# unixpickle/learn-nerf

Measured on AMD Instinct MI355X. Metric: ray-samples/s (NeRF train step: fwd + bwd + Adam, 4096 rays x 192 samples per GPU), higher is better.
Workload: dtype bf16; 1 GPU; vanilla NeRF coarse64+fine128 train step (BASELINE.json configs[1]); rays_per_gpu=4096, coarse_samples=64, fine_samples=128, global_batch_rays=4096, parallelism=dp1, precision=bf16 MFMA, fp32 accumulate/master weights

## Files before the change

### learn-nerf_amd/csrc/fused_chain.h

```cpp
#pragma once
#include <utility>

#include "common.h"
#include "fast_math.h"
#include "nerf_wgrad.h"

namespace lnrf {
using namespace nl;

typedef __bf16 bf16x8 __attribute__((ext_vector_type(8)));
typedef float f32x16 __attribute__((ext_vector_type(16)));
typedef float f32x4 __attribute__((ext_vector_type(4)));
typedef short s16x4 __attribute__((ext_vector_type(4)));


template <class F, int... I>
__device__ __forceinline__ void static_for_impl(F&& f, std::integer_sequence<int, I...>) {
  (f(std::integral_constant<int, I>{}), ...);
}
template <int N, class F>
__device__ __forceinline__ void static_for(F&& f) {
  static_for_impl(f, std::make_integer_sequence<int, N>{});
}

// ... 173 lines not shown
    w[p] = __builtin_bit_cast(unsigned, b);
  }
  return __builtin_bit_cast(bf16x8, w);
}

__device__ __forceinline__ unsigned relu_bits(const bf16x8& f0, const bf16x8& f1) {
  const uint4 a = frag_to_bits(f0), b = frag_to_bits(f1);
  const unsigned w[8] = {a.x, a.y, a.z, a.w, b.x, b.y, b.z, b.w};
  unsigned bits = 0u;
#pragma unroll
  for (int i = 0; i < 8; ++i) {
    bits |= ((w[i] & 0xFFFFu) != 0u ? 1u : 0u) << (2 * i);
    bits |= ((w[i] >> 16) != 0u ? 1u : 0u) << (2 * i + 1);
  }
  return bits;
}
template <int S>
__device__ __forceinline__ bf16x8 masked_frag(const f32x16& acc, unsigned bits, int shift) {
  bf16x8 f;
#pragma unroll
  for (int j = 0; j < 8; ++j) f[j] = (__bf16)(((bits >> (shift + 8 * S + j)) & 1u) ? acc[8 * S + j] : 0.0f);
  return f;
}

__device__ __forceinline__ void store_tile_row(float* row, int h, const f32x16& acc) {
  float* zr = row + 4 * h;
#pragma unroll
  for (int g = 0; g < 4; ++g)
    *reinterpret_cast<float4*>(zr + 8 * g) = make_float4(acc[4 * g], acc[4 * g + 1], acc[4 * g + 2], acc[4 * g + 3]);
}
__device__ __forceinline__ void stream_store(gchar* p, uint4 v) {
  u32x4 t = {v.x, v.y, v.z, v.w};
  __builtin_nontemporal_store(t, reinterpret_cast<__attribute__((address_space(1))) u32x4*>(p));
}

__device__ __forceinline__ int64_t dump_off(int slot, int64_t tile, int64_t n_tiles, int n_slots) {
  if (n_slots > 0) return (tile * n_slots + slot) * kFragBytes;
  return ((int64_t)slot * n_tiles + tile) * kFragBytes;
}
struct DumpAddr {
  char* base;
  int64_t n_tiles;
  int64_t tile;
  int c, hh;
  int n_slots;
  __device__ __forceinline__ gchar* at(int slot) const {
// ... 78 lines not shown


__device__ __forceinline__ bf16x8 tr_frag(const char* frag_even, int lane, int parity, int q) {
  const int g = lane >> 4;
  const int i = lane & 15;
  const int frag = g & 1;
  const int hk = g >> 1;
  const int qp = i >> 2, p = i & 3;
  const int slot_par = parity ^ frag;
  const int c0 = 16 * q + 8 * hk;
  const int ca = c0 + qp, cb = c0 + 4 + qp;
  const char* base = frag_even + frag * kFragBytes;
  const int offa = 256 * (ca >> 3) + 128 * (((ca >> 2) & 1) ^ slot_par) + 64 * (p & 1) + 16 * (ca & 3) + 8 * (p >> 1);
  const int offb = 256 * (cb >> 3) + 128 * (((cb >> 2) & 1) ^ slot_par) + 64 * (p & 1) + 16 * (cb & 3) + 8 * (p >> 1);
  const s16x4 lo = __builtin_amdgcn_ds_read_tr16_b64_v4i16((__attribute__((address_space(3))) s16x4*)(base + offa));
  const s16x4 hi = __builtin_amdgcn_ds_read_tr16_b64_v4i16((__attribute__((address_space(3))) s16x4*)(base + offb));
  typedef short s16x8 __attribute__((ext_vector_type(8)));
  s16x8 v;
  v[0] = lo[0]; v[1] = lo[1]; v[2] = lo[2]; v[3] = lo[3];
  v[4] = hi[0]; v[5] = hi[1]; v[6] = hi[2]; v[7] = hi[3];
  return __builtin_bit_cast(bf16x8, v);
}

template <int NXF, int NYF, int SPI, bool PLAIN = false>
struct WgStage {
  static constexpr int kWgSpi = SPI;
  static constexpr int NF = NXF + NYF;
  static constexpr int PER_WAVE = (NF + kWaves - 1) / kWaves;
  static constexpr int STEP_BYTES = NF * kFragBytes;
  static constexpr int ITER_BYTES = kWgSpi * STEP_BYTES;
  const char* x_base;
  const char* y_base;
  int x_slot0, y_slot0, x_slots, y_slots;
  int64_t t0, n_tiles;
  int64_t iter_stride, t_end;
  int wave, lane;
  uint4 rr[kWgSpi][PER_WAVE];

  __device__ __forceinline__ void load(int64_t iter) {
    const int64_t tb = t0 + iter * iter_stride;
    const int64_t tbc = tb < t_end ? tb : t0;
    const int64_t xo = dump_off(x_slot0, tbc, n_tiles, x_slots), yo = dump_off(y_slot0, tbc, n_tiles, y_slots);
    const __amdgpu_buffer_rsrc_t rx = __builtin_amdgcn_make_buffer_rsrc(const_cast<char*>(x_base) + xo, 0, 0x7FFFFFFF, 0x00020000);
    const __amdgpu_buffer_rsrc_t ry = __builtin_amdgcn_make_buffer_rsrc(const_cast<char*>(y_base) + yo, 0, 0x7FFFFFFF, 0x00020000);
#pragma unroll
    for (int u = 0; u < kWgSpi; ++u) {
      const int64_t tl = tb + u;
      const bool ok = tl < t_end;
      const int64_t ta = ok ? tl : tbc;
      const unsigned keep = ok ? 0xFFFFFFFFu : 0u;
#pragma unroll
      for (int q = 0; q < PER_WAVE; ++q) {
        int f = wave + kWaves * q;
        if constexpr (NF % kWaves != 0) f = f < NF ? f : NF - 1;
        const bool isx = f < NXF;
        const int bo = (int)(isx ? dump_off(x_slot0 + f, ta, n_tiles, x_slots) - xo
                                 : dump_off(y_slot0 + f - NXF, ta, n_tiles, y_slots) - yo);
        const u32x4 v = __builtin_amdgcn_raw_buffer_load_b128(isx ? rx : ry, bo + lane * 16, 0, PLAIN ? 0 : 2);
        rr[u][q] = make_uint4(v[0] & keep, v[1] & keep, v[2] & keep, v[3] & keep);
      }
    }
  }
  template <int B>
  __device__ __forceinline__ void write() {
#pragma unroll
    for (int u = 0; u < kWgSpi; ++u) {
#pragma unroll
      for (int q = 0; q < PER_WAVE; ++q) {
        int f = wave + kWaves * q;
        if constexpr (NF % kWaves != 0) f = f < NF ? f : NF - 1;
        *reinterpret_cast<uint4*>(&smem[B * ITER_BYTES + u * STEP_BYTES + f * kFragBytes + lane * 16]) = rr[u][q];
      }
    }
  }
};

template <int NXF, int NYF, int WI, int WO, int SPI, bool PLAIN, class PB>
__device__ __forceinline__ void wgrad_body(const PB& pb, const char* __restrict__ save,
                                           const char* __restrict__ gdump, int64_t n_tiles,
                                           WgLayout lay, float* __restrict__ slabs) {
  constexpr int NI = NXF / 2, NO = NYF / 2;
  constexpr int TI = (NI + WI - 1) / WI, TO = (NO + WO - 1) / WO;
  constexpr bool FULL_I = TI * WI == NI, FULL_O = TO * WO == NO;
  using Stage = WgStage<NXF, NYF, SPI, PLAIN>;
  constexpr int kWgSpi = SPI;
  static_assert(WI * WO == kWaves, "wave grid");
  static_assert(NXF % 2 == 0 && NYF % 2 == 0, "fragment pairs");

  const int split = blockIdx.x - pb.first_block;

  const int tid = threadIdx.x;
  const int lane = tid & 63;
  const int wave = __builtin_amdgcn_readfirstlane(tid >> 6);
  const int wi = wave / WO, wo = wave % WO;

  const int64_t per = (n_tiles + pb.n_blocks - 1) / pb.n_blocks;
  int64_t t0 = (int64_t)split * per;
  const int64_t t1 = t0 + per < n_tiles ? t0 + per : n_tiles;
  const int64_t steps = t1 > t0 ? t1 - t0 : 0;
  int64_t iters = (steps + kWgSpi - 1) / kWgSpi;
  int64_t iter_stride = kWgSpi, t_end = t1;
  if (lay.interleave) {
    t0 = (int64_t)split * kWgSpi;
    iter_stride = (int64_t)pb.n_blocks * kWgSpi;
    t_end = n_tiles;
    iters = t0 < n_tiles ? (n_tiles - t0 + iter_stride - 1) / iter_stride : 0;
  }

  Stage stg;
  stg.x_base = save;
  stg.y_base = gdump;
  stg.x_slot0 = pb.x_slot0;
  stg.y_slot0 = pb.y_slot0;
  stg.x_slots = lay.x_slots;
  stg.y_slots = lay.y_slots;
  stg.t0 = t0;
  stg.n_tiles = n_tiles;
  stg.iter_stride = iter_stride;
  stg.t_end = t_end;
  stg.wave = wave;
  stg.lane = lane;

  f32x16 acc[TI][TO];
#pragma unroll
  for (int a = 0; a < TI; ++a)
#pragma unroll
    for (int b = 0; b < TO; ++b) acc[a][b] = zero_acc();
  float bsum[TO];
#pragma unroll
  for (int b = 0; b < TO; ++b) bsum[b] = 0.0f;
  const int ypar = pb.y_slot0 & 1, xpar = pb.x_slot0 & 1;

  auto compute = [&](auto buf_) {
    constexpr int bufi = decltype(buf_)::value;
#pragma unroll
    for (int u = 0; u < kWgSpi; ++u) {
      const char* buf = smem + bufi * Stage::ITER_BYTES + u * Stage::STEP_BYTES;
#pragma unroll
      for (int q = 0; q < 2; ++q) {
        bf16x8 bf[TO];
#pragma unroll
        for (int b = 0; b < TO; ++b) {
          const int ot = wo + WO * b;
          if (FULL_O || ot < NO) {
// ... 130 lines not shown
```

### learn-nerf_amd/csrc/nerf_bwd_ls.hip

```cpp
#include "nerf_chain.h"

namespace lnrf {

constexpr int kLsWaves = 4;
constexpr int kLsThreads = kLsWaves * 64;
constexpr int kLsStages = 8;
constexpr int kLsLag = 2;
constexpr int kLsDist = kLsLag + 1;
constexpr int kLsBufs = kLsDist + 1;
constexpr int kLsTileBytes = 32 * kFragBytes;
constexpr int kLsPollOff = kLsBufs * kLsTileBytes;
constexpr int kLsLds = kLsPollOff + 5 * 256;
constexpr unsigned kLsMaxSpins = 1u << 18;
constexpr int kLsSlabWaveFloats = 16 * kSlabTileFloats + 2 * 64;
constexpr int64_t kLsSlabBlockBytes = (int64_t)kLsWaves * kLsSlabWaveFloats * (int64_t)sizeof(float);
constexpr int kLsCounterStride = 32;

struct LsJob {
  const char* packed;
  const char* save;
  char* gdump;
  unsigned* counters;
  float* slabs;
  unsigned* status;
// ... 380 lines not shown
  if (bid < n_small) {
    const int prob = bid / (kWaves * kSlabMaxTiles), w = bid / kSlabMaxTiles % kWaves, j = bid % kSlabMaxTiles;
    const WgradProblem pb = a.w[k].p[prob];
    switch (pb.shape) {
#define X(name)                                                                                                    \
  case name:                                                                                                       \
    wgrad_reduce_tile<WgShape<name>::NXF, WgShape<name>::NYF, WgShape<name>::WI, WgShape<name>::WO, NerfWgradEpi>( \
        pb, w, j, a.small_slabs[k], a.grads[k], lds);                                                              \
    break;
      LNRF_WGRAD_LS_SHAPES(X, default: X)
#undef X
    }
  } else if (bid - n_small < kLsStages * 64) {
    ls_fold_block<kSlabReduceWaves>(bid - n_small, a.ls_slabs[k], a.pipelines[k], a.grads[k], lds);
  }
}

struct BwdHeadSeq {
  static constexpr int count = bwd_cons_base(2);
  static constexpr int at(int c) { return bwd_seq(c); }
};
constexpr int kBwdHeadStages = bwd_base(2) / kStageFrags;

__global__ __launch_bounds__(kThreads) void nerf_bwd_head_kernel(
    const char* __restrict__ packed, const char* __restrict__ save, const float* __restrict__ density,
    const float* __restrict__ rgb, const float* __restrict__ g_density, const float* __restrict__ g_rgb,
    int64_t M, int64_t n_tiles, char* __restrict__ gdump, unsigned* __restrict__ zero_words, int n_zero_words) {
  const int tid = threadIdx.x;
  const int lane = tid & 63;
  const int wave = __builtin_amdgcn_readfirstlane(tid >> 6);
  const int64_t tile = (int64_t)blockIdx.x * kWaves + wave;
  for (int i = blockIdx.x * kThreads + tid; i < n_zero_words; i += gridDim.x * kThreads) zero_words[i] = 0u;
  Ring<kBwdHeadStages, BwdHeadSeq> ring;
  ring.stream = packed + kPackBwdOff;
  ring.wave = wave;
  ring.lane = lane;
  const DumpAddr gd{gdump, n_tiles, tile, lane & 31, lane >> 5, kGradTileSlots};
  bwd_chain_tile<true>(ring, gd, save, n_tiles, density, rgb, g_density, g_rgb, M, tile, lane);
}

}

using namespace lnrf;

#ifdef LNRF_TIMELINE
extern "C" int lnrf_debug_set_ls_timeline(void* buf) {
  hipError_t e = hipMemcpyToSymbol(HIP_SYMBOL(lnrf::g_ls_timeline_buf), &buf, sizeof(buf));
  return e == hipSuccess ? LNRF_OK : hip_fail(e, "hipMemcpyToSymbol(g_ls_timeline_buf)");
}
#endif

constexpr int kLsMaxPipelines = 64;
static int ls_pipelines_for_device(int need, int* out) {
  int cus = 0;
  if (int rc = cu_count(&cus)) return rc;
  *out = cus / kLsStages < kLsMaxPipelines ? cus / kLsStages : kLsMaxPipelines;
  if (*out < need) {
    set_error("layer-stationary backward: the device has too few CUs for a pipeline of 8 per model");
    return LNRF_ERR_UNSUPPORTED;
  }
  return LNRF_OK;
// ... 41 lines not shown
  a.n_jobs = 1;
  a.total_pipelines = total;
  a.job[0] = a.job[1] = ls_job(packed, save, scratch, m, total);
  hipError_t e = hipMemsetAsync(a.job[0].counters, 0, kLsCounterBytes, st);
  if (e != hipSuccess) return hip_fail(e, "hipMemsetAsync(counters)");
  hipLaunchKernelGGL(nerf_bwd_ls_kernel, dim3((unsigned)(total * kLsStages)), dim3(kLsThreads), kLsLds, st, a);
  LNRF_LAUNCH_CHECK();
  hipLaunchKernelGGL(nerf_ls_reduce_kernel, dim3(kLsStages * 64), dim3(256), 0, st, (const float*)a.job[0].slabs, total, grads);
  LNRF_LAUNCH_CHECK();
  return LNRF_OK;
}

namespace {
struct LsModel {
  const void* packed;
  const void* save;
  const float *density, *rgb, *g_density, *g_rgb;
  int64_t m;
  void* scratch;
  float* grads;
};
}

static int ls_backward(const LsModel* mdl, int n_models, int phases, hipStream_t st) {
  constexpr int kHeadLds = kRingBytes + round_up(kBiasFloats * 4, 1024);
  int total = 0;
  int rc = ls_pipelines_for_device(n_models, &total);
  if (!rc) rc = set_max_dynamic_lds(nerf_bwd_head_kernel, kHeadLds);
  if (!rc) rc = set_max_dynamic_lds(nerf_bwd_ls_kernel, kLsLds);
  if (rc) return rc;
  int pipes[2] = {total, 0};
  if (n_models == 2) {
    const double share = (double)mdl[0].m / (double)(mdl[0].m + mdl[1].m);
    pipes[0] = (int)(total * share + 0.5);
    if (pipes[0] < 1) pipes[0] = 1;
    if (pipes[0] > total - 1) pipes[0] = total - 1;
    pipes[1] = total - pipes[0];
  }
  LsArgs a;
  a.n_jobs = n_models;
  a.total_pipelines = total;
  for (int k = 0; k < n_models; ++k) {
    const LsModel& md = mdl[k];
    const LsJob& j = a.job[k] = ls_job(md.packed, md.save, md.scratch, md.m, pipes[k]);
    if (phases & 1) {
      hipLaunchKernelGGL(nerf_bwd_head_kernel, dim3((unsigned)(j.n_tiles / kWaves)), dim3(kThreads), kHeadLds, st, j.packed,
                         j.save, md.density, md.rgb, md.g_density, md.g_rgb, md.m, j.n_tiles, j.gdump, j.counters,
                         (phases & 2) ? (int)(kLsCounterBytes / sizeof(unsigned)) : 0);
      LNRF_LAUNCH_CHECK();
    }
    if ((phases & 3) == 2) {
      hipError_t e = hipMemsetAsync(j.counters, 0, kLsCounterBytes, st);
      if (e != hipSuccess) return hip_fail(e, "hipMemsetAsync(counters)");
    }
  }
  if (n_models == 1) a.job[1] = a.job[0];
  if (phases & 2) {
    hipLaunchKernelGGL(nerf_bwd_ls_kernel, dim3((unsigned)(total * kLsStages)), dim3(kLsThreads), kLsLds, st, a);
    LNRF_LAUNCH_CHECK();
  }
  if (!(phases & 4)) return LNRF_OK;
  LsFoldArgs fold;
  for (int k = 0; k < n_models; ++k) {
    const LsModel& md = mdl[k];
    const LsJob& j = a.job[k];
    const WgradList w = wgrad_list_ls_finish(j.n_tiles);
    float* small_slabs = ls_small_slabs(md.scratch, md.m);
    rc = launch_nerf_wgrad(w, md.save, md.scratch, j.n_tiles, md.grads, st, WgLayout{kSaveTileSlots, kGradTileSlots, 1},
                           small_slabs, false, false);
    if (rc) return rc;
    fold.w[k] = w.args;
    fold.small_slabs[k] = small_slabs;
    fold.ls_slabs[k] = j.slabs;
    fold.grads[k] = md.grads;
    fold.pipelines[k] = pipes[k];
  }
  if (n_models == 1) {
    fold.w[1] = fold.w[0]; fold.small_slabs[1] = fold.small_slabs[0]; fold.ls_slabs[1] = fold.ls_slabs[0];
    fold.grads[1] = fold.grads[0]; fold.pipelines[1] = fold.pipelines[0];
  }
  const int gx = fold.w[0].n_problems * kWaves * kSlabMaxTiles + kLsStages * 64;
  hipLaunchKernelGGL(nerf_ls_fold_kernel, dim3((unsigned)gx, (unsigned)n_models), dim3(64 * kSlabReduceWaves), 0, st, fold);
  LNRF_LAUNCH_CHECK();
  return LNRF_OK;
}

extern "C" int lnrf_nerf_mlp_bwd_ls(const lnrf_nerf_shape* shape, const void* packed, const void* save,
                                    const float* density, const float* rgb, const float* g_density,
                                    const float* g_rgb, int64_t m, void* scratch, float* grads, int32_t phases,
                                    lnrf_stream_t stream) {
  LNRF_REQUIRE_NERF_SHAPE(shape);
  LNRF_CHECK_ARG(packed && save && density && rgb && g_density && g_rgb && scratch && grads, "null pointer");
  LNRF_CHECK_ARG(m >= 0, "bad m");
  if (m == 0) return LNRF_OK;
  LNRF_CHECK_ARG(phases >= 1 && phases <= 7, "phases: bit 0 head, bit 1 pipeline, bit 2 small problems + fold");
  const LsModel md{packed, save, density, rgb, g_density, g_rgb, m, scratch, grads};
  return ls_backward(&md, 1, phases, as_stream(stream));
}

extern "C" int lnrf_nerf_mlp_bwd_ls2(const lnrf_nerf_shape* shape, const void* packed_a, const void* save_a,
                                     const float* density_a, const float* rgb_a, const float* g_density_a,
                                     const float* g_rgb_a, int64_t m_a, void* scratch_a, float* grads_a,
                                     const void* packed_b, const void* save_b, const float* density_b,
                                     const float* rgb_b, const float* g_density_b, const float* g_rgb_b, int64_t m_b,
                                     void* scratch_b, float* grads_b, int32_t phases, lnrf_stream_t stream) {
  LNRF_REQUIRE_NERF_SHAPE(shape);
  LNRF_CHECK_ARG(packed_a && save_a && density_a && rgb_a && g_density_a && g_rgb_a && scratch_a && grads_a, "null pointer");
  LNRF_CHECK_ARG(packed_b && save_b && density_b && rgb_b && g_density_b && g_rgb_b && scratch_b && grads_b, "null pointer");
  LNRF_CHECK_ARG(m_a > 0 && m_b > 0, "both models need evaluations (use lnrf_nerf_mlp_bwd_ls for one)");
  const LsModel md[2] = {{packed_a, save_a, density_a, rgb_a, g_density_a, g_rgb_a, m_a, scratch_a, grads_a},
                         {packed_b, save_b, density_b, rgb_b, g_density_b, g_rgb_b, m_b, scratch_b, grads_b}};
  LNRF_CHECK_ARG(phases >= 1 && phases <= 7, "phases: bit 0 head, bit 1 pipeline, bit 2 small problems + fold");
  return ls_backward(md, 2, phases, as_stream(stream));
}
```

### learn-nerf_amd/csrc/nerf_chain.h

```cpp
#pragma once
#include "fused_chain.h"

namespace lnrf {

template <class Put>
__device__ __forceinline__ void x_encode(const float (&px)[3], int h, Put put) {
  static_for<4>([&](auto ks_) {
    constexpr int ks = decltype(ks_)::value;
#pragma unroll
    for (int pp = 0; pp < 4; ++pp) {
      const int p = 4 * ks + pp;
      float s = 0.0f, co = 0.0f;
      if (p < kXPairs) {
        const int pg = kXPairs * h + p;
        const int cd = pg / kXFreqs, f = pg - kXFreqs * cd;
        const float v = cd == 0 ? px[0] : (cd == 1 ? px[1] : px[2]);
        sincos_pe(v * (float)(1 << f), &s, &co);
      }
      put(ks_, 2 * pp, s);
      put(ks_, 2 * pp + 1, co);
    }
  });
}

// ... 12 lines not shown
        else return xe[ks - 16];
      },
      epi);
}
template <int S, class RING, class Epi>
__device__ __forceinline__ void trunk_layer_split(RING& ring, int h, const bf16x8 (&xe_hi)[4], const bf16x8 (&xe_lo)[4],
                                                  const bf16x8 (&inh)[16], const bf16x8 (&inl)[16], Epi epi) {
  chain_layer_split<fwd_cons_base(S), fwd_nk(S), fwd_no(S)>(
      ring, [&](auto o_) { return bias_acc(fwd_bias_base(S) + 32 * decltype(o_)::value, h); },
      [&](auto k_) -> bf16x8 {
        constexpr int ks = decltype(k_)::value;
        if constexpr (S == 0) return xe_hi[ks];
        else if constexpr (ks < 16) return inh[ks];
        else return xe_hi[ks - 16];
      },
      [&](auto k_) -> bf16x8 {
        constexpr int ks = decltype(k_)::value;
        if constexpr (S == 0) return xe_lo[ks];
        else if constexpr (ks < 16) return inl[ks];
        else return xe_lo[ks - 16];
      },
      epi);
}
template <int O>
__device__ __forceinline__ void masked_out_tile(const f32x16& acc, const uint4& mk, bf16x8 (&out)[16], const DumpAddr& gd,
                                                int slot0) {
  const unsigned mb = mask_word(mk, O);
  out[2 * O] = masked_frag<0>(acc, mb, 16 * (O & 1));
  out[2 * O + 1] = masked_frag<1>(acc, mb, 16 * (O & 1));
  gd.store(slot0 + 2 * O, frag_to_bits(out[2 * O]));
  gd.store(slot0 + 2 * O + 1, frag_to_bits(out[2 * O + 1]));
}
template <int C0, int L, class RING>
__device__ __forceinline__ void hidden_back(RING& ring, bf16x8 (&in)[16], bf16x8 (&out)[16], const uint4& mk,
                                            const DumpAddr& gd) {
  chain_layer<C0, 16, 8>(
      ring, [&](auto) { return zero_acc(); }, [&](auto k_) -> bf16x8 { return in[decltype(k_)::value]; },
      [&](auto o_, const f32x16& acc) { masked_out_tile<decltype(o_)::value>(acc, mk, out, gd, grad_dy_slot(L - 1)); });
}

struct BwdSeq {
  static constexpr int count = kBwdUsed;
  static constexpr int at(int c) { return bwd_seq(c); }
};
constexpr int kBwdStages = kBwdFrags / kStageFrags;

template <bool HEAD_ONLY = false, class RING>
__device__ __forceinline__ void bwd_chain_tile(RING& ring, const DumpAddr& gd, const char* __restrict__ save,
                                               int64_t save_tiles, const float* __restrict__ density,
                                               const float* __restrict__ rgb, const float* __restrict__ g_density,
                                               const float* __restrict__ g_rgb, int64_t M, int64_t tile, int lane) {
  const int c = lane & 31, h = lane >> 5;
  const int64_t m = tile * kTileCols + c;
  const bool valid = m < M;

  float gy11[3] = {0, 0, 0}, gy9 = 0.0f;
  if (valid && h == 0) {
#pragma unroll
    for (int k = 0; k < 3; ++k) {
      const float y = rgb[m * 3 + k];
      gy11[k] = g_rgb[m * 3 + k] * (1.0f - y * y);
    }
    gy9 = g_density[m] * -expm1f(-density[m]);
  }
  uint4 relu_mask[9];
#pragma unroll
  for (int i = HEAD_ONLY ? 8 : 0; i < 9; ++i)
    relu_mask[i] = *mask_at(save, kSaveMask + i, tile, save_tiles, kSaveTileSlots, lane);
  __syncthreads();
  ring.prologue();
  LNRF_TL_STAMP(ring);

  bf16x8 a0[16], a1[16];

  bf16x8 dy11 = zero_frag();
  dy11[0] = (__bf16)gy11[0];
  dy11[1] = (__bf16)gy11[1];
  dy11[2] = (__bf16)gy11[2];
  gd.store(kGradDy11, frag_to_bits(dy11));
  gd.store(kGradDy11 + 1, frag_to_bits(zero_frag()));

  chain_layer<bwd_cons_base(0), bwd_nk(0), bwd_no(0)>(
      ring, [&](auto) { return zero_acc(); }, [&](auto) -> bf16x8 { return dy11; },
      [&](auto o_, const f32x16& acc) {
        masked_out_tile<decltype(o_)::value>(acc, relu_mask[8], a0, gd, kGradDy10m);
      });
  bf16x8 dlogit = zero_frag();
  dlogit[0] = (__bf16)gy9;
  gd.store(kGradDy10m + 8, frag_to_bits(dlogit));
  gd.store(kGradDy10m + 9, frag_to_bits(zero_frag()));

  chain_layer<bwd_cons_base(1), bwd_nk(1), bwd_no(1)>(
      ring, [&](auto) { return zero_acc(); },
      [&](auto k_) -> bf16x8 {
        constexpr int ks = decltype(k_)::value;
        if constexpr (ks < 8) return a0[ks];
        else return dlogit;
      },
      [&](auto o_, const f32x16& acc) {
        constexpr int o = decltype(o_)::value;
        a1[2 * o] = acc_to_frag<0, false>(acc);
        a1[2 * o + 1] = acc_to_frag<1, false>(acc);
        gd.store(grad_dy_slot(8) + 2 * o, frag_to_bits(a1[2 * o]));
        gd.store(grad_dy_slot(8) + 2 * o + 1, frag_to_bits(a1[2 * o + 1]));
      });

  if constexpr (HEAD_ONLY) return;
  static_assert(bwd_nk(2) == 16 && bwd_no(2) == 8, "hidden_back");
  static_for<8>([&](auto i_) {
    constexpr int TT = 2 + decltype(i_)::value, l = bwd_dense(TT);
    if constexpr (TT % 2 == 0) hidden_back<bwd_cons_base(TT), l>(ring, a1, a0, relu_mask[l - 1], gd);
    else hidden_back<bwd_cons_base(TT), l>(ring, a0, a1, relu_mask[l - 1], gd);
  });
}

int launch_nerf_wgrad(const WgradList& list, const void* xbuf, const void* ybuf, int64_t n_tiles, float* grads,
                      hipStream_t stream, WgLayout lay, float* slabs, bool plain_loads = false,
                      bool fold = true);

int64_t ls_scratch_bytes(int64_t m);
float* ls_small_slabs(void* scratch, int64_t m);
int launch_ls_pipeline(const void* packed, const void* save, void* scratch, int64_t m, float* grads, hipStream_t stream);

}
```

### learn-nerf_amd/csrc/nerf_mlp.hip

```cpp
#include "nerf_chain.h"

namespace lnrf {

constexpr int kFusedLds = kRingBytes + round_up(kBiasFloats * 4, 1024);
#ifdef LNRF_TIMELINE
__device__ unsigned long long* g_timeline_buf = nullptr;
#endif

struct FwdSeq {
  static constexpr int count = kFwdUsed;
  static constexpr int at(int c) { return fwd_seq(c); }
};

constexpr int kFwdStages = kFwdFrags / kStageFrags;

template <bool SAVE, bool FROM_RAYS, bool HMASKS = true>
__global__ __launch_bounds__(kThreads) void nerf_fwd_kernel(
    const char* __restrict__ packed, const float* __restrict__ xin_g, const float* __restrict__ din_g,
    const float* __restrict__ rays, int64_t ray_stride, const float* __restrict__ ts, int T, int64_t M,
    int64_t n_tiles, float* __restrict__ density, float* __restrict__ rgb, char* __restrict__ save) {
  const auto [lane, wave, c, h, tile, m, valid] = tile_ctx<kWaves>(M);

  stage_bias<kThreads>(packed + kPackBiasOff, kBiasFloats);
  float px[3] = {0, 0, 0}, pd[3] = {0, 0, 0};
// ... 249 lines not shown
__global__ __launch_bounds__(kThreads) void nerf_bwd_chain_kernel(
    const char* __restrict__ packed, const char* __restrict__ save, const float* __restrict__ density,
    const float* __restrict__ rgb, const float* __restrict__ g_density, const float* __restrict__ g_rgb,
    int64_t M, int64_t n_tiles, char* __restrict__ gdump) {
  const auto [lane, wave, c, h, tile, m, valid] = tile_ctx<kWaves>(M);

  Ring<kBwdStages, BwdSeq> ring;
  ring.stream = packed + kPackBwdOff;
  ring.wave = wave;
  ring.lane = lane;
#ifdef LNRF_TIMELINE
  ring.tl.buf = g_timeline_buf + 16 * 1024;
  ring.tl.n = 0;
  ring.tl.on = g_timeline_buf != nullptr && blockIdx.x == gridDim.x / 2;
  ring.tl.stamp();
#endif
  const DumpAddr gd{gdump, n_tiles, tile, c, h, kGradTileSlots};
  bwd_chain_tile(ring, gd, save, n_tiles, density, rgb, g_density, g_rgb, M, tile, lane);
}

template <bool PLAIN>
__global__ __launch_bounds__(kThreads) void nerf_wgrad_kernel(WgradArgs args, const char* __restrict__ save,
                                                              const char* __restrict__ gdump, int64_t n_tiles,
                                                              WgLayout lay, float* __restrict__ slabs) {
  WgradProblem pb = args.p[0];
#pragma unroll
  for (int i = 1; i < kMaxProblems; ++i)
    if (i < args.n_problems && (int)blockIdx.x >= args.p[i].first_block) pb = args.p[i];
  switch (pb.shape) {
#define X(name, id, NXF, NYF, WI, WO, SPI) \
  case name: wgrad_body<NXF, NYF, WI, WO, SPI, PLAIN>(pb, save, gdump, n_tiles, lay, slabs); break;
    LNRF_WGRAD_SHAPES(X, default: X)
#undef X
  }
}

__global__ __launch_bounds__(64 * kSlabReduceWaves) void nerf_wgrad_reduce_kernel(WgradArgs args,
                                                                                 const float* __restrict__ slabs,
                                                                                 float* __restrict__ grads) {
  __shared__ float lds[(kSlabReduceWaves - 1) * 17 * 64];
  const int prob = blockIdx.x / (kWaves * kSlabMaxTiles), w = blockIdx.x / kSlabMaxTiles % kWaves, j = blockIdx.x % kSlabMaxTiles;
  const WgradProblem pb = args.p[prob];
  switch (pb.shape) {
#define X(name, id, NXF, NYF, WI, WO, SPI) \
  case name: wgrad_reduce_tile<NXF, NYF, WI, WO, NerfWgradEpi>(pb, w, j, slabs, grads, lds); break;
    LNRF_WGRAD_SHAPES(X, default: X)
#undef X
  }
}

__global__ void nerf_pack_kernel(const float* __restrict__ params, char* __restrict__ packed) {
  constexpr int64_t units_f = (int64_t)kFwdFrags * 64, units_b = (int64_t)kBwdFrags * 64;
  constexpr int64_t total = units_f + units_b + kBiasFloats;
  for (int64_t u = (int64_t)blockIdx.x * blockDim.x + threadIdx.x; u < total; u += (int64_t)gridDim.x * blockDim.x) {
// ... 153 lines not shown
  LNRF_LAUNCH_CHECK();
  return LNRF_OK;
}

extern "C" int lnrf_nerf_mlp_bwd_chain(const lnrf_nerf_shape* shape, const void* packed, const void* save,
                                       const float* density, const float* rgb, const float* g_density,
                                       const float* g_rgb, int64_t m, void* scratch, lnrf_stream_t stream) {
  LNRF_REQUIRE_NERF_SHAPE(shape);
  LNRF_CHECK_ARG(packed && save && density && rgb && g_density && g_rgb && scratch, "null pointer");
  LNRF_CHECK_ARG(m >= 0, "bad m");
  if (m == 0) return LNRF_OK;
  const int64_t n_tiles = padded_tiles(m);
  hipStream_t st = as_stream(stream);
  int rc = set_max_dynamic_lds(nerf_bwd_chain_kernel, kFusedLds);
  if (rc) return rc;
  hipLaunchKernelGGL(nerf_bwd_chain_kernel, dim3((unsigned)((n_tiles + kWaves - 1) / kWaves)), dim3(kThreads),
                     kFusedLds, st, (const char*)packed, (const char*)save, density, rgb, g_density, g_rgb, m,
                     n_tiles, (char*)scratch);
  LNRF_LAUNCH_CHECK();
  return LNRF_OK;
}

int lnrf::launch_nerf_wgrad(const WgradList& list, const void* xbuf, const void* ybuf, int64_t n_tiles, float* grads,
                            hipStream_t stream, WgLayout lay, float* slabs, bool plain, bool fold) {
  LNRF_CHECK_ARG(slabs != nullptr && list.blocks <= kWgradMaxBlocks, "needs slabs, and holds at most kWgradMaxBlocks of them");
  const int lds = 2 * 2 * 36 * kFragBytes;
  const dim3 grid((unsigned)list.blocks), block(kThreads);
  int rc = plain ? set_max_dynamic_lds(nerf_wgrad_kernel<true>, lds) : set_max_dynamic_lds(nerf_wgrad_kernel<false>, lds);
  if (rc) return rc;
  if (plain)
    hipLaunchKernelGGL(nerf_wgrad_kernel<true>, grid, block, lds, stream, list.args, (const char*)xbuf,
                       (const char*)ybuf, n_tiles, lay, slabs);
  else
    hipLaunchKernelGGL(nerf_wgrad_kernel<false>, grid, block, lds, stream, list.args, (const char*)xbuf,
                       (const char*)ybuf, n_tiles, lay, slabs);
  LNRF_LAUNCH_CHECK();
  if (fold) {
    hipLaunchKernelGGL(nerf_wgrad_reduce_kernel, dim3((unsigned)(list.args.n_problems * kWaves * kSlabMaxTiles)),
                       dim3(64 * kSlabReduceWaves), 0, stream, list.args, (const float*)slabs, grads);
    LNRF_LAUNCH_CHECK();
  }
  return LNRF_OK;
}

extern "C" int lnrf_nerf_mlp_bwd_weights(const lnrf_nerf_shape* shape, const void* save, void* scratch,
                                         int64_t m, float* grads, lnrf_stream_t stream) {
  LNRF_REQUIRE_NERF_SHAPE(shape);
  LNRF_CHECK_ARG(save && scratch && grads, "null pointer");
  LNRF_CHECK_ARG(m >= 0, "bad m");
  if (m == 0) return LNRF_OK;
  const int64_t n_tiles = padded_tiles(m);
  float* slabs = reinterpret_cast<float*>(reinterpret_cast<char*>(scratch) + grad_dump_bytes(m));
  constexpr int64_t kPlainFrom = 16384;
  return launch_nerf_wgrad(wgrad_list_split(n_tiles), save, scratch, n_tiles, grads, as_stream(stream),
                           WgLayout{kSaveTileSlots, kGradTileSlots}, slabs, n_tiles >= kPlainFrom);
}

#ifdef LNRF_TIMELINE
// ... 6 lines not shown
```

### learn-nerf_amd/csrc/nerf_wgrad.h

```cpp
#pragma once
#include "nerf_layout.h"

namespace lnrf {
using namespace nl;

constexpr int kSlabMaxTiles = 9, kSlabMaxTO = 4;
constexpr int kSlabTileFloats = 64 * 16;
constexpr int kSlabWaveFloats = kSlabMaxTiles * kSlabTileFloats + kSlabMaxTO * 64;
constexpr int64_t kSlabBlockBytes = (int64_t)kWaves * kSlabWaveFloats * (int64_t)sizeof(float);
constexpr int kWgradMaxBlocks = 512;
constexpr int64_t kWgradSlabBytes = kWgradMaxBlocks * kSlabBlockBytes;

#define LNRF_WGRAD_SHAPES(X, X_ELSE)                                                                      \
  X(WG_HIDDEN, 0, 16, 16, 4, 2, 2)                                          \
  X(WG_Z_DY10M, 1, 16, 10, 4, 2, 2)                                                        \
  X(WG_XEMB, 2, 4, 16, 2, 4, 3)                                             \
  X(WG_DEMB_DY10M, 3, 2, 10, 1, 8, 5)                                                  \
  X(WG_DIR9, 5, 18, 8, 4, 2, 2)                                                     \
  X(WG_ZD_DY10M, 6, 18, 10, 4, 2, 2)                                             \
  X(WG_XEMB_DY0_DY5, 7, 4, 32, 2, 4, 2)                                          \
  X_ELSE(WG_H128_DY3, 4, 8, 2, 4, 2, 6)
#define LNRF_WGRAD_LS_SHAPES(X, X_ELSE) X(WG_XEMB_DY0_DY5) X(WG_ZD_DY10M) X_ELSE(WG_H128_DY3)

enum WgradShape : int {
#define X(name, id, nxf, nyf, wi, wo, spi) name = id,
  LNRF_WGRAD_SHAPES(X, X)
#undef X
};
template <WgradShape S>
struct WgShape;
#define X(name, id, nxf, nyf, wi, wo, spi)                                              \
  template <>                                                                           \
  struct WgShape<name> {                                                                \
    static constexpr int NXF = nxf, NYF = nyf, WI = wi, WO = wo, SPI = spi;             \
    static constexpr int TI = (nxf / 2 + wi - 1) / wi, TO = (nyf / 2 + wo - 1) / wo;  \
  };
LNRF_WGRAD_SHAPES(X, X)
#undef X

enum { ROW_HIDDEN = 0, ROW_XEMB = 1, ROW_DEMB = 2, ROW_Z_DEMB = 3 };
enum { COL_256 = 0, COL_DY10M = 1, COL_DY11 = 2, COL_EXPLICIT = 3, COL_DY0_DY5 = 4 };
struct WgradProblem {
  WgradShape shape;
  int x_slot0;
  int y_slot0;
  int dense;
  int row_map;
  int row_off;
  int col_map;
  int do_bias;
  int first_block, n_blocks;
  int w_off, b_off, out_dim, n_rows;
};
constexpr int kMaxProblems = 13;
struct WgradArgs {
  WgradProblem p[kMaxProblems];
  int n_problems;
};

struct NerfWgradEpi {
  static NL_HD void cols(const WgradProblem& pb, int ot, int colr, int& out_idx, int& out_dim, int64_t& w_off,
                         int64_t& b_off) {
    int dense_w = pb.dense;
    if (pb.col_map == COL_DY10M) {
      if (ot < 4) { out_idx = 32 * ot + colr; out_dim = 128; dense_w = 10; }
      else if (colr == 0 && pb.row_map != ROW_DEMB) { out_idx = 0; out_dim = 1; dense_w = 9; }
    } else if (pb.col_map == COL_DY0_DY5) {
      out_idx = 32 * (ot & 7) + colr; out_dim = 256;
      if (ot >= 8) {
        w_off = dense_w_off(5) + 256 * 256;
        b_off = -1;
        return;
      }
      dense_w = 0;
    } else if (pb.col_map == COL_DY11) {
      if (colr < 3) { out_idx = colr; out_dim = 3; }
    } else if (pb.col_map == COL_EXPLICIT) {
      if (32 * ot + colr < pb.out_dim) out_idx = 32 * ot + colr;
      out_dim = pb.out_dim;
      w_off = pb.w_off;
// ... 62 lines not shown
  }
};

struct WgradList {
  WgradArgs args;
  int blocks = 0;
  int64_t cap;
  explicit WgradList(int64_t n_tiles) : cap((n_tiles + 5) / 6) { args.n_problems = 0; }

  WgradProblem& add(int want, WgradShape shape, int xs, int ys, int dense, int row_map, int row_off, int col_map,
                    int do_bias) {
    WgradProblem& p = args.p[args.n_problems++];
    p = WgradProblem{shape, xs, ys, dense, row_map, row_off, col_map, do_bias, blocks, (int)(want < cap ? want : cap),
                     0, 0, 0, 0};
    blocks += p.n_blocks;
    return p;
  }
  void hidden(int want, int l, int do_bias) {
    add(want, WG_HIDDEN, kSaveH + (l - 1) * 16, grad_dy_slot(l), l, ROW_HIDDEN, 0, COL_256, do_bias);
  }
  void xemb_dy0_dy5(int want, int do_bias) {
    add(want, WG_XEMB_DY0_DY5, kSaveXin, grad_dy_slot(0), 0, ROW_XEMB, 0, COL_DY0_DY5, do_bias);
  }
  void zd_dy10m(int want) { add(want, WG_ZD_DY10M, kSaveZ, kGradDy10m, 10, ROW_Z_DEMB, 0, COL_DY10M, 1); }
  void h10_dy11(int want) { add(want, WG_H128_DY3, kSaveH10, kGradDy11, 11, ROW_HIDDEN, 0, COL_DY11, 1); }
  void explicit_at(int want, WgradShape shape, int xs, int ys, int out_dim, int n_rows, int w_off, int b_off) {
    WgradProblem& p = add(want, shape, xs, ys, 0, ROW_HIDDEN, 0, COL_EXPLICIT, 1);
    p.w_off = w_off; p.b_off = b_off; p.out_dim = out_dim; p.n_rows = n_rows;
  }
};

inline WgradList wgrad_list_split(int64_t n_tiles) {
  WgradList w(n_tiles);
  for (int l = 1; l <= 8; ++l) w.hidden(l <= 4 ? 48 : 47, l, 1);
  w.add(39, WG_Z_DY10M, kSaveZ, kGradDy10m, 10, ROW_HIDDEN, 0, COL_DY10M, 1);
  w.add(30, WG_XEMB, kSaveXin, grad_dy_slot(0), 0, ROW_XEMB, 0, COL_256, 1);
  w.add(30, WG_XEMB, kSaveXin, grad_dy_slot(5), 5, ROW_XEMB, 256, COL_256, 0);
  w.add(18, WG_DEMB_DY10M, kSaveDin, kGradDy10m, 10, ROW_DEMB, 256, COL_DY10M, 0);
  w.h10_dy11(15);
  return w;
}
inline WgradList wgrad_list_ls_finish(int64_t n_tiles) {
  WgradList w(n_tiles);
  w.xemb_dy0_dy5(256 * 36 / 74, 1);
  w.zd_dy10m(256 * 28 / 74);
  w.h10_dy11(256 * 10 / 74);
  return w;
}
inline WgradList wgrad_list_ref_trunk(int64_t n_tiles) {
  WgradList w(n_tiles);
  w.xemb_dy0_dy5(256, 1);
  return w;
}
inline WgradList wgrad_list_ref_normal(int64_t n_tiles) {
  WgradList w(n_tiles);
  for (int l = 1; l <= 8; ++l) w.hidden(28, l, 0);
  w.xemb_dy0_dy5(32, 0);
  return w;
}
inline WgradList wgrad_list_ref_dir(int64_t n_tiles) {
  WgradList w(n_tiles);
  w.explicit_at(200, WG_DIR9, kDirSaveXin, kDirGradDy9, kDirHidden, kDirIn, kDirW9, kDirB9);
  w.explicit_at(56, WG_H128_DY3, kDirSaveH, kDirGradDy10, 3, kDirHidden, kDirW10, kDirB10);
  return w;
}

}
```

Before: 186.7 million ray-samples/s.

## Recompute head output-gradients inside wgrad instead of dumping them to memory

In the two-model LS backward path, the head kernel no longer writes the dy11 and dy10m gradient fragments to the global dump. The wgrad kernel instead recomputes them per tile from rgb, density and their gradients, using a small MFMA against LDS-staged weights and saved relu masks. This removes a global write and reread of those fragments in exchange for extra loads and MFMA work on producer waves inside wgrad. The single-model path keeps dumping the head fragments but its wgrad list now also uses the producing shapes.

```diff
diff --git a/learn-nerf_amd/csrc/fused_chain.h b/learn-nerf_amd/csrc/fused_chain.h
--- a/learn-nerf_amd/csrc/fused_chain.h
+++ b/learn-nerf_amd/csrc/fused_chain.h
@@ -219,6 +219,9 @@
   for (int j = 0; j < 8; ++j) f[j] = (__bf16)(((bits >> (shift + 8 * S + j)) & 1u) ? acc[8 * S + j] : 0.0f);
   return f;
 }
+
+__device__ __forceinline__ float head_gy11(float g_rgb, float y) { return g_rgb * (1.0f - y * y); }
+__device__ __forceinline__ float head_gy9(float g_density, float density) { return g_density * -expm1f(-density); }
 
 __device__ __forceinline__ void store_tile_row(float* row, int h, const f32x16& acc) {
   float* zr = row + 4 * h;
@@ -343,13 +346,17 @@
   return __builtin_bit_cast(bf16x8, v);
 }
 
-template <int NXF, int NYF, int SPI, bool PLAIN = false>
+template <int NXF, int NYF, int SPI, bool PLAIN = false, int GEN = WG_LOADS_DY>
 struct WgStage {
   static constexpr int kWgSpi = SPI;
   static constexpr int NF = NXF + NYF;
-  static constexpr int PER_WAVE = (NF + kWaves - 1) / kWaves;
+  static constexpr int NLD = GEN != WG_LOADS_DY ? NXF : NF;
+  static constexpr int PER_WAVE = (NLD + kWaves - 1) / kWaves;
   static constexpr int STEP_BYTES = NF * kFragBytes;
   static constexpr int ITER_BYTES = kWgSpi * STEP_BYTES;
+  static constexpr int kWLdsOff = 2 * ITER_BYTES;
+  static constexpr int kProdIn = GEN == WG_MAKES_DY10M ? 8 : 6;
+  static_assert(GEN == WG_LOADS_DY || (SPI <= kWaves && NYF == (GEN == WG_MAKES_DY10M ? 2 * bwd_no(0) + 2 : 2)), "producer");
   const char* x_base;
   const char* y_base;
   int x_slot0, y_slot0, x_slots, y_slots;
@@ -357,6 +364,9 @@
   int64_t iter_stride, t_end;
   int wave, lane;
   uint4 rr[kWgSpi][PER_WAVE];
+  WgProducer prod;
+  float pin[kProdIn];
+  uint2 pmask;
 
   __device__ __forceinline__ void load(int64_t iter) {
     const int64_t tb = t0 + iter * iter_stride;
@@ -373,14 +383,38 @@
 #pragma unroll
       for (int q = 0; q < PER_WAVE; ++q) {
         int f = wave + kWaves * q;
-        if constexpr (NF % kWaves != 0) f = f < NF ? f : NF - 1;
-        const bool isx = f < NXF;
+        if constexpr (NLD % kWaves != 0) f = f < NLD ? f : NLD - 1;
+        const bool isx = GEN != WG_LOADS_DY || f < NXF;
         const int bo = (int)(isx ? dump_off(x_slot0 + f, ta, n_tiles, x_slots) - xo
                                  : dump_off(y_slot0 + f - NXF, ta, n_tiles, y_slots) - yo);
         const u32x4 v = __builtin_amdgcn_raw_buffer_load_b128(isx ? rx : ry, bo + lane * 16, 0, PLAIN ? 0 : 2);
         rr[u][q] = make_uint4(v[0] & keep, v[1] & keep, v[2] & keep, v[3] & keep);
       }
     }
+    if constexpr (GEN != WG_LOADS_DY) {
+      const int pu = kWaves - 1 - wave;
+      if (pu < kWgSpi) {
+        const int64_t tl = tb + pu;
+        const bool ok = tl < t_end;
+        const int64_t ta = ok ? tl : tbc;
+        const int64_t m = ta * kTileCols + (lane & 31);
+        const bool live = ok && lane < 32 && m < prod.M;
+        const int64_t ma = live ? m : 0;
+        if constexpr (GEN == WG_MAKES_DY10M)
+          pmask = *reinterpret_cast<const uint2*>(mask_at(x_base, kSaveMask + 8, ta, n_tiles, x_slots, lane));
+#pragma unroll
+        for (int k = 0; k < 3; ++k) {
+          const float y = prod.rgb[ma * 3 + k], g = prod.g_rgb[ma * 3 + k];
+          pin[k] = live ? y : 0.0f;
+          pin[3 + k] = live ? g : 0.0f;
+        }
+        if constexpr (GEN == WG_MAKES_DY10M) {
+          const float d = prod.density[ma], g = prod.g_density[ma];
+          pin[6] = live ? d : 0.0f;
+          pin[7] = live ? g : 0.0f;
+        }
+      }
+    }
   }
   template <int B>
   __device__ __forceinline__ void write() {
@@ -389,21 +423,54 @@
 #pragma unroll
       for (int q = 0; q < PER_WAVE; ++q) {
         int f = wave + kWaves * q;
-        if constexpr (NF % kWaves != 0) f = f < NF ? f : NF - 1;
+        if constexpr (NLD % kWaves != 0) f = f < NLD ? f : NLD - 1;
         *reinterpret_cast<uint4*>(&smem[B * ITER_BYTES + u * STEP_BYTES + f * kFragBytes + lane * 16]) = rr[u][q];
       }
     }
+    if constexpr (GEN != WG_LOADS_DY) {
+      __builtin_amdgcn_sched_barrier(0);
+      const int pu = kWaves - 1 - wave;
+      if (pu < kWgSpi) {
+        const int c = lane & 31, hh = lane >> 5;
+        char* ybuf = &smem[B * ITER_BYTES + pu * STEP_BYTES + NXF * kFragBytes];
+        auto put = [&](int f, const bf16x8& v) {
+          *reinterpret_cast<uint4*>(ybuf + f * kFragBytes + dump_lane_off(y_slot0 + f, c, hh)) = frag_to_bits(v);
+        };
+        bf16x8 dy11 = zero_frag();
+#pragma unroll
+        for (int k = 0; k < 3; ++k) dy11[k] = (__bf16)head_gy11(pin[3 + k], pin[k]);
+        if constexpr (GEN == WG_MAKES_DY11) {
+          put(0, dy11);
+          put(1, zero_frag());
+        } else {
+          static_for<bwd_no(0)>([&](auto o_) {
+            constexpr int o = decltype(o_)::value;
+            const bf16x8 a = bits_to_frag(*reinterpret_cast<const uint4*>(&smem[kWLdsOff + o * kFragBytes + lane * 16]));
+            const f32x16 acc = __builtin_amdgcn_mfma_f32_32x32x16_bf16(a, dy11, zero_acc(), 0, 0, 0);
+            const unsigned mb = mask_word(make_uint4(pmask.x, pmask.y, 0u, 0u), o);
+            put(2 * o, masked_frag<0>(acc, mb, 16 * (o & 1)));
+            put(2 * o + 1, masked_frag<1>(acc, mb, 16 * (o & 1)));
+            __builtin_amdgcn_sched_barrier(0);
+          });
+          bf16x8 dlogit = zero_frag();
+          dlogit[0] = (__bf16)head_gy9(pin[7], pin[6]);
+          put(2 * bwd_no(0), dlogit);
+          put(2 * bwd_no(0) + 1, zero_frag());
+        }
+      }
+      __builtin_amdgcn_sched_barrier(0);
+    }
   }
 };
 
-template <int NXF, int NYF, int WI, int WO, int SPI, bool PLAIN, class PB>
+template <int NXF, int NYF, int WI, int WO, int SPI, bool PLAIN, int GEN = WG_LOADS_DY, class PB>
 __device__ __forceinline__ void wgrad_body(const PB& pb, const char* __restrict__ save,
                                            const char* __restrict__ gdump, int64_t n_tiles,
-                                           WgLayout lay, float* __restrict__ slabs) {
+                                           WgLayout lay, float* __restrict__ slabs, const WgProducer& prod = WgProducer{}) {
   constexpr int NI = NXF / 2, NO = NYF / 2;
   constexpr int TI = (NI + WI - 1) / WI, TO = (NO + WO - 1) / WO;
   constexpr bool FULL_I = TI * WI == NI, FULL_O = TO * WO == NO;
-  using Stage = WgStage<NXF, NYF, SPI, PLAIN>;
+  using Stage = WgStage<NXF, NYF, SPI, PLAIN, GEN>;
   constexpr int kWgSpi = SPI;
   static_assert(WI * WO == kWaves, "wave grid");
   static_assert(NXF % 2 == 0 && NYF % 2 == 0, "fragment pairs");
@@ -441,6 +508,14 @@
   stg.t_end = t_end;
   stg.wave = wave;
   stg.lane = lane;
+  if constexpr (GEN != WG_LOADS_DY) stg.prod = prod;
+  if constexpr (GEN == WG_MAKES_DY10M) {
+    if (wave < bwd_no(0)) {
+      const char* src = prod.packed + kPackBwdOff + (int64_t)bwd_seq(bwd_cons_base(0) + wave) * kFragBytes + lane * 16;
+      *reinterpret_cast<uint4*>(&smem[Stage::kWLdsOff + wave * kFragBytes + lane * 16]) = *reinterpret_cast<const uint4*>(src);
+    }
+    __syncthreads();
+  }
 
   f32x16 acc[TI][TO];
 #pragma unroll
diff --git a/learn-nerf_amd/csrc/nerf_bwd_ls.hip b/learn-nerf_amd/csrc/nerf_bwd_ls.hip
--- a/learn-nerf_amd/csrc/nerf_bwd_ls.hip
+++ b/learn-nerf_amd/csrc/nerf_bwd_ls.hip
@@ -426,6 +426,7 @@
 };
 constexpr int kBwdHeadStages = bwd_base(2) / kStageFrags;
 
+template <bool LEAN>
 __global__ __launch_bounds__(kThreads) void nerf_bwd_head_kernel(
     const char* __restrict__ packed, const char* __restrict__ save, const float* __restrict__ density,
     const float* __restrict__ rgb, const float* __restrict__ g_density, const float* __restrict__ g_rgb,
@@ -440,7 +441,7 @@
   ring.wave = wave;
   ring.lane = lane;
   const DumpAddr gd{gdump, n_tiles, tile, lane & 31, lane >> 5, kGradTileSlots};
-  bwd_chain_tile<true>(ring, gd, save, n_tiles, density, rgb, g_density, g_rgb, M, tile, lane);
+  bwd_chain_tile<true, !LEAN>(ring, gd, save, n_tiles, density, rgb, g_density, g_rgb, M, tile, lane);
 }
 
 }
@@ -528,11 +529,12 @@
 };
 }
 
-static int ls_backward(const LsModel* mdl, int n_models, int phases, hipStream_t st) {
+static int ls_backward(const LsModel* mdl, int n_models, int phases, bool lean_head, hipStream_t st) {
   constexpr int kHeadLds = kRingBytes + round_up(kBiasFloats * 4, 1024);
   int total = 0;
   int rc = ls_pipelines_for_device(n_models, &total);
-  if (!rc) rc = set_max_dynamic_lds(nerf_bwd_head_kernel, kHeadLds);
+  auto head = lean_head ? nerf_bwd_head_kernel<true> : nerf_bwd_head_kernel<false>;
+  if (!rc) rc = set_max_dynamic_lds(head, kHeadLds);
   if (!rc) rc = set_max_dynamic_lds(nerf_bwd_ls_kernel, kLsLds);
   if (rc) return rc;
   int pipes[2] = {total, 0};
@@ -550,7 +552,7 @@
     const LsModel& md = mdl[k];
     const LsJob& j = a.job[k] = ls_job(md.packed, md.save, md.scratch, md.m, pipes[k]);
     if (phases & 1) {
-      hipLaunchKernelGGL(nerf_bwd_head_kernel, dim3((unsigned)(j.n_tiles / kWaves)), dim3(kThreads), kHeadLds, st, j.packed,
+      hipLaunchKernelGGL(head, dim3((unsigned)(j.n_tiles / kWaves)), dim3(kThreads), kHeadLds, st, j.packed,
                          j.save, md.density, md.rgb, md.g_density, md.g_rgb, md.m, j.n_tiles, j.gdump, j.counters,
                          (phases & 2) ? (int)(kLsCounterBytes / sizeof(unsigned)) : 0);
       LNRF_LAUNCH_CHECK();
@@ -573,7 +575,8 @@
     const WgradList w = wgrad_list_ls_finish(j.n_tiles);
     float* small_slabs = ls_small_slabs(md.scratch, md.m);
     rc = launch_nerf_wgrad(w, md.save, md.scratch, j.n_tiles, md.grads, st, WgLayout{kSaveTileSlots, kGradTileSlots, 1},
-                           small_slabs, false, false);
+                           small_slabs, false, false,
+                           WgProducer{(const char*)md.packed, md.density, md.rgb, md.g_density, md.g_rgb, md.m});
     if (rc) return rc;
     fold.w[k] = w.args;
     fold.small_slabs[k] = small_slabs;
@@ -601,7 +604,7 @@
   if (m == 0) return LNRF_OK;
   LNRF_CHECK_ARG(phases >= 1 && phases <= 7, "phases: bit 0 head, bit 1 pipeline, bit 2 small problems + fold");
   const LsModel md{packed, save, density, rgb, g_density, g_rgb, m, scratch, grads};
-  return ls_backward(&md, 1, phases, as_stream(stream));
+  return ls_backward(&md, 1, phases, false, as_stream(stream));
 }
 
 extern "C" int lnrf_nerf_mlp_bwd_ls2(const lnrf_nerf_shape* shape, const void* packed_a, const void* save_a,
@@ -617,5 +620,5 @@
   const LsModel md[2] = {{packed_a, save_a, density_a, rgb_a, g_density_a, g_rgb_a, m_a, scratch_a, grads_a},
                          {packed_b, save_b, density_b, rgb_b, g_density_b, g_rgb_b, m_b, scratch_b, grads_b}};
   LNRF_CHECK_ARG(phases >= 1 && phases <= 7, "phases: bit 0 head, bit 1 pipeline, bit 2 small problems + fold");
-  return ls_backward(md, 2, phases, as_stream(stream));
-}
+  return ls_backward(md, 2, phases, true, as_stream(stream));
+}
diff --git a/learn-nerf_amd/csrc/nerf_chain.h b/learn-nerf_amd/csrc/nerf_chain.h
--- a/learn-nerf_amd/csrc/nerf_chain.h
+++ b/learn-nerf_amd/csrc/nerf_chain.h
@@ -58,14 +58,16 @@
       },
       epi);
 }
-template <int O>
+template <int O, bool DUMP = true>
 __device__ __forceinline__ void masked_out_tile(const f32x16& acc, const uint4& mk, bf16x8 (&out)[16], const DumpAddr& gd,
                                                 int slot0) {
   const unsigned mb = mask_word(mk, O);
   out[2 * O] = masked_frag<0>(acc, mb, 16 * (O & 1));
   out[2 * O + 1] = masked_frag<1>(acc, mb, 16 * (O & 1));
-  gd.store(slot0 + 2 * O, frag_to_bits(out[2 * O]));
-  gd.store(slot0 + 2 * O + 1, frag_to_bits(out[2 * O + 1]));
+  if constexpr (DUMP) {
+    gd.store(slot0 + 2 * O, frag_to_bits(out[2 * O]));
+    gd.store(slot0 + 2 * O + 1, frag_to_bits(out[2 * O + 1]));
+  }
 }
 template <int C0, int L, class RING>
 __device__ __forceinline__ void hidden_back(RING& ring, bf16x8 (&in)[16], bf16x8 (&out)[16], const uint4& mk,
@@ -81,7 +83,7 @@
 };
 constexpr int kBwdStages = kBwdFrags / kStageFrags;
 
-template <bool HEAD_ONLY = false, class RING>
+template <bool HEAD_ONLY = false, bool DUMP_HEAD = true, class RING>
 __device__ __forceinline__ void bwd_chain_tile(RING& ring, const DumpAddr& gd, const char* __restrict__ save,
                                                int64_t save_tiles, const float* __restrict__ density,
                                                const float* __restrict__ rgb, const float* __restrict__ g_density,
@@ -95,9 +97,9 @@
 #pragma unroll
     for (int k = 0; k < 3; ++k) {
       const float y = rgb[m * 3 + k];
-      gy11[k] = g_rgb[m * 3 + k] * (1.0f - y * y);
+      gy11[k] = head_gy11(g_rgb[m * 3 + k], y);
     }
-    gy9 = g_density[m] * -expm1f(-density[m]);
+    gy9 = head_gy9(g_density[m], density[m]);
   }
   uint4 relu_mask[9];
 #pragma unroll
@@ -113,18 +115,22 @@
   dy11[0] = (__bf16)gy11[0];
   dy11[1] = (__bf16)gy11[1];
   dy11[2] = (__bf16)gy11[2];
-  gd.store(kGradDy11, frag_to_bits(dy11));
-  gd.store(kGradDy11 + 1, frag_to_bits(zero_frag()));
+  if constexpr (DUMP_HEAD) {
+    gd.store(kGradDy11, frag_to_bits(dy11));
+    gd.store(kGradDy11 + 1, frag_to_bits(zero_frag()));
+  }
 
   chain_layer<bwd_cons_base(0), bwd_nk(0), bwd_no(0)>(
       ring, [&](auto) { return zero_acc(); }, [&](auto) -> bf16x8 { return dy11; },
       [&](auto o_, const f32x16& acc) {
-        masked_out_tile<decltype(o_)::value>(acc, relu_mask[8], a0, gd, kGradDy10m);
+        masked_out_tile<decltype(o_)::value, DUMP_HEAD>(acc, relu_mask[8], a0, gd, kGradDy10m);
       });
   bf16x8 dlogit = zero_frag();
   dlogit[0] = (__bf16)gy9;
-  gd.store(kGradDy10m + 8, frag_to_bits(dlogit));
-  gd.store(kGradDy10m + 9, frag_to_bits(zero_frag()));
+  if constexpr (DUMP_HEAD) {
+    gd.store(kGradDy10m + 8, frag_to_bits(dlogit));
+    gd.store(kGradDy10m + 9, frag_to_bits(zero_frag()));
+  }
 
   chain_layer<bwd_cons_base(1), bwd_nk(1), bwd_no(1)>(
       ring, [&](auto) { return zero_acc(); },
@@ -152,7 +158,8 @@
 
 int launch_nerf_wgrad(const WgradList& list, const void* xbuf, const void* ybuf, int64_t n_tiles, float* grads,
                       hipStream_t stream, WgLayout lay, float* slabs, bool plain_loads = false,
-                      bool fold = true);
+                      bool fold = true,
+                      const WgProducer& prod = WgProducer{});
 
 int64_t ls_scratch_bytes(int64_t m);
 float* ls_small_slabs(void* scratch, int64_t m);
diff --git a/learn-nerf_amd/csrc/nerf_mlp.hip b/learn-nerf_amd/csrc/nerf_mlp.hip
--- a/learn-nerf_amd/csrc/nerf_mlp.hip
+++ b/learn-nerf_amd/csrc/nerf_mlp.hip
@@ -295,14 +295,14 @@
 template <bool PLAIN>
 __global__ __launch_bounds__(kThreads) void nerf_wgrad_kernel(WgradArgs args, const char* __restrict__ save,
                                                               const char* __restrict__ gdump, int64_t n_tiles,
-                                                              WgLayout lay, float* __restrict__ slabs) {
+                                                              WgLayout lay, float* __restrict__ slabs, WgProducer prod) {
   WgradProblem pb = args.p[0];
 #pragma unroll
   for (int i = 1; i < kMaxProblems; ++i)
     if (i < args.n_problems && (int)blockIdx.x >= args.p[i].first_block) pb = args.p[i];
   switch (pb.shape) {
 #define X(name, id, NXF, NYF, WI, WO, SPI) \
-  case name: wgrad_body<NXF, NYF, WI, WO, SPI, PLAIN>(pb, save, gdump, n_tiles, lay, slabs); break;
+  case name: wgrad_body<NXF, NYF, WI, WO, SPI, PLAIN, wg_produces(name)>(pb, save, gdump, n_tiles, lay, slabs, prod); break;
     LNRF_WGRAD_SHAPES(X, default: X)
 #undef X
   }
@@ -502,18 +502,22 @@
 }
 
 int lnrf::launch_nerf_wgrad(const WgradList& list, const void* xbuf, const void* ybuf, int64_t n_tiles, float* grads,
-                            hipStream_t stream, WgLayout lay, float* slabs, bool plain, bool fold) {
+                            hipStream_t stream, WgLayout lay, float* slabs, bool plain, bool fold, const WgProducer& prod) {
   LNRF_CHECK_ARG(slabs != nullptr && list.blocks <= kWgradMaxBlocks, "needs slabs, and holds at most kWgradMaxBlocks of them");
+  for (int i = 0; i < list.args.n_problems; ++i)
+    LNRF_CHECK_ARG(wg_produces(list.args.p[i].shape) == WG_LOADS_DY ||
+                       (prod.packed && prod.density && prod.rgb && prod.g_density && prod.g_rgb && prod.M > 0),
+                   "a producing shape needs the head's inputs");
   const int lds = 2 * 2 * 36 * kFragBytes;
   const dim3 grid((unsigned)list.blocks), block(kThreads);
   int rc = plain ? set_max_dynamic_lds(nerf_wgrad_kernel<true>, lds) : set_max_dynamic_lds(nerf_wgrad_kernel<false>, lds);
   if (rc) return rc;
   if (plain)
     hipLaunchKernelGGL(nerf_wgrad_kernel<true>, grid, block, lds, stream, list.args, (const char*)xbuf,
-                       (const char*)ybuf, n_tiles, lay, slabs);
+                       (const char*)ybuf, n_tiles, lay, slabs, prod);
   else
     hipLaunchKernelGGL(nerf_wgrad_kernel<false>, grid, block, lds, stream, list.args, (const char*)xbuf,
-                       (const char*)ybuf, n_tiles, lay, slabs);
+                       (const char*)ybuf, n_tiles, lay, slabs, prod);
   LNRF_LAUNCH_CHECK();
   if (fold) {
     hipLaunchKernelGGL(nerf_wgrad_reduce_kernel, dim3((unsigned)(list.args.n_problems * kWaves * kSlabMaxTiles)),
diff --git a/learn-nerf_amd/csrc/nerf_wgrad.h b/learn-nerf_amd/csrc/nerf_wgrad.h
--- a/learn-nerf_amd/csrc/nerf_wgrad.h
+++ b/learn-nerf_amd/csrc/nerf_wgrad.h
@@ -19,8 +19,10 @@
   X(WG_DIR9, 5, 18, 8, 4, 2, 2)                                                     \
   X(WG_ZD_DY10M, 6, 18, 10, 4, 2, 2)                                             \
   X(WG_XEMB_DY0_DY5, 7, 4, 32, 2, 4, 2)                                          \
+  X(WG_ZD_RE10M, 8, 18, 10, 4, 2, 2)      \
+  X(WG_H128_RE11, 9, 8, 2, 4, 2, 6)                            \
   X_ELSE(WG_H128_DY3, 4, 8, 2, 4, 2, 6)
-#define LNRF_WGRAD_LS_SHAPES(X, X_ELSE) X(WG_XEMB_DY0_DY5) X(WG_ZD_DY10M) X_ELSE(WG_H128_DY3)
+#define LNRF_WGRAD_LS_SHAPES(X, X_ELSE) X(WG_XEMB_DY0_DY5) X(WG_ZD_RE10M) X_ELSE(WG_H128_RE11)
 
 enum WgradShape : int {
 #define X(name, id, nxf, nyf, wi, wo, spi) name = id,
@@ -37,6 +39,8 @@
   };
 LNRF_WGRAD_SHAPES(X, X)
 #undef X
+enum { WG_LOADS_DY = 0, WG_MAKES_DY10M = 1, WG_MAKES_DY11 = 2 };
+constexpr int wg_produces(WgradShape s) { return s == WG_ZD_RE10M ? WG_MAKES_DY10M : (s == WG_H128_RE11 ? WG_MAKES_DY11 : WG_LOADS_DY); }
 
 enum { ROW_HIDDEN = 0, ROW_XEMB = 1, ROW_DEMB = 2, ROW_Z_DEMB = 3 };
 enum { COL_256 = 0, COL_DY10M = 1, COL_DY11 = 2, COL_EXPLICIT = 3, COL_DY0_DY5 = 4 };
@@ -56,6 +60,11 @@
 struct WgradArgs {
   WgradProblem p[kMaxProblems];
   int n_problems;
+};
+struct WgProducer {
+  const char* packed = nullptr;
+  const float *density = nullptr, *rgb = nullptr, *g_density = nullptr, *g_rgb = nullptr;
+  int64_t M = 0;
 };
 
 struct NerfWgradEpi {
@@ -164,8 +173,12 @@
   void xemb_dy0_dy5(int want, int do_bias) {
     add(want, WG_XEMB_DY0_DY5, kSaveXin, grad_dy_slot(0), 0, ROW_XEMB, 0, COL_DY0_DY5, do_bias);
   }
-  void zd_dy10m(int want) { add(want, WG_ZD_DY10M, kSaveZ, kGradDy10m, 10, ROW_Z_DEMB, 0, COL_DY10M, 1); }
-  void h10_dy11(int want) { add(want, WG_H128_DY3, kSaveH10, kGradDy11, 11, ROW_HIDDEN, 0, COL_DY11, 1); }
+  void zd_dy10m(int want, bool remake = false) {
+    add(want, remake ? WG_ZD_RE10M : WG_ZD_DY10M, kSaveZ, kGradDy10m, 10, ROW_Z_DEMB, 0, COL_DY10M, 1);
+  }
+  void h10_dy11(int want, bool remake = false) {
+    add(want, remake ? WG_H128_RE11 : WG_H128_DY3, kSaveH10, kGradDy11, 11, ROW_HIDDEN, 0, COL_DY11, 1);
+  }
   void explicit_at(int want, WgradShape shape, int xs, int ys, int out_dim, int n_rows, int w_off, int b_off) {
     WgradProblem& p = add(want, shape, xs, ys, 0, ROW_HIDDEN, 0, COL_EXPLICIT, 1);
     p.w_off = w_off; p.b_off = b_off; p.out_dim = out_dim; p.n_rows = n_rows;
@@ -185,8 +198,8 @@
 inline WgradList wgrad_list_ls_finish(int64_t n_tiles) {
   WgradList w(n_tiles);
   w.xemb_dy0_dy5(256 * 36 / 74, 1);
-  w.zd_dy10m(256 * 28 / 74);
-  w.h10_dy11(256 * 10 / 74);
+  w.zd_dy10m(256 * 28 / 74, true);
+  w.h10_dy11(256 * 10 / 74, true);
   return w;
 }
 inline WgradList wgrad_list_ref_trunk(int64_t n_tiles) {
```

Result: slower. 177.2 million ray-samples/s (-5.1%).
